# apachepinot/pinot

Measured on NVIDIA B200. Metric: scanned rows/sec for filter+groupby(3 dims,4 aggs) @1/2/4/8 B200; %HBM BW, higher is better.
Workload: dtype f64

## Files before the change

### include/pinot_b200.h

```cpp
#ifndef PINOT_B200_H
#define PINOT_B200_H

#include <stddef.h>
#include <stdint.h>

#ifdef __cplusplus
extern "C" {
#endif

#define PB_OK 0
#define PB_ERR_INVALID (-1)
#define PB_ERR_UNSUPPORTED (-2)
#define PB_ERR_CUDA (-3)
#define PB_ERR_OOM (-4)
#define PB_ERR_STATE (-5)

enum { PB_INT = 0, PB_LONG = 1, PB_FLOAT = 2, PB_DOUBLE = 3, PB_STRING = 4 };

enum { PB_AGG_COUNT = 0, PB_AGG_SUM = 1, PB_AGG_MIN = 2, PB_AGG_MAX = 3, PB_AGG_AVG = 4, PB_AGG_DISTINCTCOUNT = 5 };

enum {
  PB_F_AND = 0, PB_F_OR = 1, PB_F_NOT = 2, PB_F_MATCH_ALL = 3, PB_F_EMPTY = 4,
  PB_F_SCAN_DICT_RANGE = 5,
  PB_F_SCAN_DICT_SET = 6,
// ... 125 lines not shown

int pb_segment_group_remap(pb_segment_group_handle g, const char* column, int32_t segment_index, const int32_t** remap, int32_t* n);

int pb_query_execute(pb_segment_group_handle g, const pb_segment_query* seg_queries, const pb_query_desc* q,
                     pb_result_handle* out);

int32_t pb_result_num_tables(pb_result_handle r);
int64_t pb_result_num_groups(pb_result_handle r, int32_t table);
const int32_t* pb_result_group_dict_ids(pb_result_handle r, int32_t table, int32_t gb);
const void* pb_result_group_key_values(pb_result_handle r, int32_t table, int32_t gb, int32_t* stored_type,
                                       int32_t* entry_bytes);
const double* pb_result_double(pb_result_handle r, int32_t table, int32_t agg);
const int64_t* pb_result_long(pb_result_handle r, int32_t table, int32_t agg);
const int64_t* pb_result_distinct_offsets(pb_result_handle r, int32_t table, int32_t agg);
const int32_t* pb_result_distinct_dict_ids(pb_result_handle r, int32_t table, int32_t agg);
const int64_t* pb_result_distinct_values(pb_result_handle r, int32_t table, int32_t agg);
const pb_exec_stats* pb_result_stats(pb_result_handle r, int32_t table);
double pb_result_device_ms(pb_result_handle r);
double pb_result_scan_kernel_ms(pb_result_handle r);
int pb_result_phase_ms(pb_result_handle r, double* filter_kernel_ms, double* agg_kernel_ms);
int32_t pb_result_kernel_launches(pb_result_handle r);
double pb_result_comm_ms(pb_result_handle r);
int32_t pb_result_in_place_columns(pb_result_handle r);
int pb_result_host_timing(pb_result_handle r, double* out8);
void pb_result_free(pb_result_handle r);

int pb_result_device_buffer(pb_result_handle r, int32_t which, int32_t agg, void** device_ptr, int64_t* num_elements);
int pb_result_merge_gathered(pb_result_handle r, const void* gathered_device_ptr, int32_t n_ranks);
int pb_result_finalize(pb_result_handle r);
void* pb_result_stream(pb_result_handle r);
int pb_result_wait(pb_result_handle r);

int pb_host_register(const void* ptr, size_t bytes);
int pb_host_unregister(const void* ptr);

#ifdef __cplusplus
}
#endif
#endif
```

### pinot_b200/csrc/pb_device.cuh

```cuda
#pragma once
#include <cuda_runtime.h>
#include <stdint.h>

#define PB_NTHREADS 256
#define PB_NWARPS 8
#define PB_CHUNK_DOCS 1024
#define PB_NSTAGE 2
#define PB_MAX_LEAVES 16
#define PB_MAX_NODES 32
#define PB_MAX_GROUP_BY 16
#define PB_MAX_AGGS 16
#define PB_MAX_SCAN_SLOTS 8
#define PB_MAX_AGG_FILTERS 8
#define PB_MAX_AF_LEAVES 16
#define PB_MAX_AF_NODES 48
#define PB_SPARSE_MAX 128
#define PB_OUT_CAP 256
#define PB_CAND_CAP 512
#define PB_SET_SMEM_BYTES 8192

enum { L_TRUE = 0, L_FALSE = 1, L_DICT_RANGE = 2, L_DICT_SET = 3, L_RAW_RANGE_I = 4, L_RAW_RANGE_F = 5,
       L_RAW_SET = 6, L_BITMAP = 7 };
enum { N_LEAF = 0, N_AND = 1, N_OR = 2, N_NOT = 3 };
enum { T_KEYLESS = 0, T_DENSE = 1, T_HASH = 2 };
// ... 105 lines not shown
  unsigned long long* docs_matched;
  uint32_t* first_doc;
  uint32_t num_groups_limit;
  uint32_t limit_active;
};

struct DevQuery {
  int32_t n_segs;
  int32_t n_group_by;
  int32_t n_aggs;
  int32_t table_mode;
  int32_t agg_op[PB_MAX_AGGS];
  int32_t agg_filter_of[PB_MAX_AGGS];
  int32_t n_agg_filters;
  int32_t pad_f;
  int32_t slot_off[PB_MAX_SCAN_SLOTS];
  int32_t stage_bytes;
  int32_t set_cache_bytes;
  int32_t use_tma;
  int32_t generic;
  uint64_t n_units;
  uint64_t n_docs_total;
  int32_t match_all;
  int32_t pad_p;
  int32_t sparse_max;
  int32_t cand_bytes;
  uint64_t unit_lo;
  int32_t phase;
  int32_t st_slots;
  int32_t st_replicas;
  int32_t out_cap, cand_cap;
  uint64_t st_min_docs;
  uint32_t* match_list;
  unsigned long long* match_count;
  const unsigned int* any_limit;
  const DevSegQuery* segs;
  DevTable* tables;
};

__device__ __forceinline__ uint32_t pb_bswap32(uint32_t x) { return __byte_perm(x, 0, 0x0123); }

__device__ __forceinline__ long long pb_enc_f64(double v) {
  long long b = __double_as_longlong(v);
  return b >= 0 ? b : (b ^ 0x7fffffffffffffffLL);
}
__host__ __device__ __forceinline__ double pb_dec_f64(long long e) {
  long long b = e >= 0 ? e : (e ^ 0x7fffffffffffffffLL);
// ... 895 lines not shown
          for (uint32_t b0 = 0; b0 < n_pass; b0 += 32) {
            const uint32_t idx = b0 + (uint32_t)lane;
            bool alive = idx < n_pass;
            const uint32_t off = alive ? (uint32_t)cl[idx] : 0u;
            const uint32_t doc = (uint32_t)unit_doc0 + off;
            for (int i = 0; i < n_cand_leaves; i++) {
              if (alive) alive = pb_leaf_test_doc(sq.leaves[H->flat_leaf[H->n_dense + i]], set_cache, doc);
              if (!__any_sync(0xffffffffu, alive)) break;
            }
            const uint32_t bal = __ballot_sync(0xffffffffu, alive);
            if (bal) {
              const uint32_t n = (uint32_t)__popc(bal);
              if (out_n + n > OUT_CAP) flush_out();
              if (alive) ob[out_n + __popc(bal & lt)] = gunit0 + off;
              out_n += n;
              matched += n;
            }
          }
        }
        __syncwarp();
      }
    }
    flush_out();
    if (lane == 0 && matched) pb_red_add_u64(Q.tables[sq.table].docs_matched, matched);
  }
}

#define PB_AGG_MAX_SEGS_SMEM 1024

template <int MIN_CTAS>
__global__ void __launch_bounds__(PB_NTHREADS, MIN_CTAS) pb_agg_kernel(const __grid_constant__ DevQuery Q) {
  extern __shared__ __align__(128) uint8_t smem_raw[];
  const int tid = threadIdx.x, lane = tid & 31, warp = tid >> 5;
  __shared__ unsigned long long s_doc_base[PB_AGG_MAX_SEGS_SMEM + 1];
  __shared__ unsigned long long s_red_u64[PB_NWARPS];
  __shared__ double s_red_f64[PB_NWARPS];
  __shared__ long long s_red_i64[PB_NWARPS];
  __shared__ int s_table0;
  const int n_segs = Q.n_segs;
  const int n_smem = n_segs < PB_AGG_MAX_SEGS_SMEM ? n_segs : PB_AGG_MAX_SEGS_SMEM;
  for (int i = tid; i < n_smem; i += PB_NTHREADS) s_doc_base[i] = Q.segs[i].doc_base;
  KeylessAcc ka;
  ka.sum = nullptr; ka.mm = nullptr; ka.cnt = nullptr;
  const long long ENC_POS_INF = 0x7ff0000000000000LL;
  const long long ENC_NEG_INF = (long long)0xfff0000000000000ULL ^ 0x7fffffffffffffffLL;
  const bool keyless = Q.table_mode == T_KEYLESS;
  if (keyless) {
// ... 192 lines not shown
    for (int a = 0; a < Q.n_aggs; a++) {
      if (st.fc_of[a] >= 0) {
        unsigned long long fc = 0;
        for (uint32_t r = 0; r < R; r++) { SmemTable z = st; z.base = smem0 + r * (uint32_t)rep_bytes; fc += pb_sh_ld_u32(z.fcnt(st.fc_of[a], i)); }
        if (fc) pb_red_add_u64(&t.fcnt[a][i], fc);
      }
      if (st.acc_of[a] < 0) continue;
      const int op = Q.agg_op[a];
      if (op == 1 || op == 4) {
        double v = 0.0;
        for (uint32_t r = 0; r < R; r++) { SmemTable z = st; z.base = smem0 + r * (uint32_t)rep_bytes; v += __longlong_as_double((long long)pb_sh_ld_u64(z.acc(st.acc_of[a], i))); }
        pb_red_add_f64(&t.sum[a][i], v);
      } else {
        long long m = 0x7fffffffffffffffLL;
        for (uint32_t r = 0; r < R; r++) { SmemTable z = st; z.base = smem0 + r * (uint32_t)rep_bytes; const long long o = (long long)pb_sh_ld_u64(z.acc(st.acc_of[a], i)); m = o < m ? o : m; }
        if (m != 0x7fffffffffffffffLL) pb_red_min_s64(&t.mm[a][i], m);
      }
    }
  }
}

struct DevRowKey { uint32_t off, bits; uint64_t mult; const int32_t* remap; };
struct DevRowAgg { uint32_t off, width, type, exact_int; };
struct DevRowSeg {
  const uint32_t* rows;
  uint64_t doc_base;
  int32_t table, pad;
  DevRowKey keys[PB_MAX_GROUP_BY];
  DevRowAgg aggs[PB_MAX_AGGS];
};
#define PB_ROWS_SMEM_SEGS 16

template <int RW>
__global__ void __launch_bounds__(PB_AGG_SMEM_THREADS, 1) pb_agg_rows_kernel(const __grid_constant__ DevQuery Q, const DevRowSeg* __restrict__ gsegs) {
  extern __shared__ __align__(128) uint8_t smem_raw[];
  __shared__ DevRowSeg s_segs[PB_ROWS_SMEM_SEGS];
  __shared__ unsigned long long s_doc_base[PB_AGG_MAX_SEGS_SMEM + 1];
  const int tid = threadIdx.x, warp = tid >> 5;
  const int n_segs = Q.n_segs, nG = Q.n_group_by, nA = Q.n_aggs;
  const int n_smem = n_segs < PB_AGG_MAX_SEGS_SMEM ? n_segs : PB_AGG_MAX_SEGS_SMEM;
  for (int i = tid; i < n_smem; i += PB_AGG_SMEM_THREADS) s_doc_base[i] = gsegs[i].doc_base;
  const bool segs_in_smem = n_segs <= PB_ROWS_SMEM_SEGS;
  if (segs_in_smem) {
    const uint32_t* src = reinterpret_cast<const uint32_t*>(gsegs);
    uint32_t* dst = reinterpret_cast<uint32_t*>(s_segs);
    for (int i = tid; i < (int)(sizeof(DevRowSeg) / 4) * n_segs; i += PB_AGG_SMEM_THREADS) dst[i] = src[i];
  }
  const DevRowSeg* segs = segs_in_smem ? s_segs : gsegs;
  const unsigned long long n = Q.match_all ? Q.n_docs_total : *Q.match_count;
  const uint32_t S = (uint32_t)Q.st_slots, R = (uint32_t)(Q.st_replicas > 0 ? Q.st_replicas : 1);
  SmemTable st;
  st.S = S;
  int n_acc = 0;
  for (int a = 0; a < PB_MAX_AGGS; a++) {
    const int op = a < nA ? Q.agg_op[a] : 0;
    st.acc_of[a] = (a < nA && op >= 1 && op <= 4) ? (int8_t)n_acc++ : (int8_t)-1;
    st.fc_of[a] = -1;
  }
  st.n_fc = 0;
  const size_t rep_bytes = pb_smem_table_bytes(S, 0, n_acc);
  const uint32_t smem0 = pb_smem_u32(smem_raw);
  st.base = smem0 + ((uint32_t)warp & (R - 1)) * (uint32_t)rep_bytes;
  const bool use_smem = S > 0 && n >= Q.st_min_docs;
  if (use_smem) {
    for (uint32_t r = 0; r < R; r++) {
      SmemTable z = st; z.base = smem0 + r * (uint32_t)rep_bytes;
      for (uint32_t i = tid; i < S; i += PB_AGG_SMEM_THREADS) pb_sh_st_u32(z.cnt(i), 0u);
      for (int a = 0; a < nA; a++) {
        if (st.acc_of[a] < 0) continue;
        const unsigned long long init = (Q.agg_op[a] == 1 || Q.agg_op[a] == 4) ? 0ull : 0x7fffffffffffffffull;
        for (uint32_t i = tid; i < S; i += PB_AGG_SMEM_THREADS) pb_sh_st_u64(z.acc(st.acc_of[a], i), init);
      }
    }
  }
  __syncthreads();

  auto process = [&](unsigned long long gdoc, const uint32_t (&w)[RW], const DevRowSeg& sg) {
    auto field = [&](uint32_t off, uint32_t bits) -> uint32_t {
      const uint32_t wi = off >> 5, sh = off & 31u;
      uint32_t hi = w[0], lo = RW > 1 ? w[1 % RW] : 0u;
#pragma unroll
      for (int k = 1; k < RW; k++) if (wi == (uint32_t)k) { hi = w[k]; lo = k + 1 < RW ? w[(k + 1) % RW] : 0u; }
      return __funnelshift_l(lo, hi, sh) >> (32u - bits);
    };
    uint64_t slot = 0;
    for (int j = 0; j < nG; j++) {
      const DevRowKey& k = sg.keys[j];
      uint32_t id = field(k.off, k.bits);
      if (k.remap) id = (uint32_t)__ldg(k.remap + id);
      slot += (uint64_t)id * k.mult;
    }
    auto value_of = [&](int a) -> double {
      const DevRowAgg& g = sg.aggs[a];
      const uint32_t w0 = field(g.off, 32u);
      if (g.width == 4) return g.type == 2 ? (double)__uint_as_float(w0) : (double)(int32_t)w0;
      const unsigned long long u = ((unsigned long long)w0 << 32) | field(g.off + 32u, 32u);
      return g.type == 3 ? __longlong_as_double((long long)u) : (double)(long long)u;
    };
    auto ivalue_of = [&](int a) -> long long {
      const DevRowAgg& g = sg.aggs[a];
      const uint32_t w0 = field(g.off, 32u);
      if (g.width == 4) return (long long)(int32_t)w0;
      return (long long)(((unsigned long long)w0 << 32) | field(g.off + 32u, 32u));
    };
    if (use_smem) {
      const uint32_t sl = (uint32_t)slot;
      pb_sh_add_u32(st.cnt(sl), 1u);
// ... 39 lines not shown
  };
  auto seg_of = [&](unsigned long long gdoc) -> int {
    int lo = 0, hi = n_segs - 1;
    while (lo < hi) {
      const int mid = (lo + hi + 1) >> 1;
      const unsigned long long b = mid < PB_AGG_MAX_SEGS_SMEM ? s_doc_base[mid] : gsegs[mid].doc_base;
      if (b <= gdoc) lo = mid; else hi = mid - 1;
    }
    return lo;
  };
  auto load_row = [&](const DevRowSeg& sg, unsigned long long gdoc, uint32_t (&w)[RW]) {
    const uint32_t* __restrict__ row = sg.rows + (gdoc - sg.doc_base) * (unsigned long long)RW;
    if (RW == 2) { const uint2 v = __ldg(reinterpret_cast<const uint2*>(row)); w[0] = v.x; w[1 % RW] = v.y; }
    else {
#pragma unroll
      for (int q4 = 0; q4 < RW / 4; q4++) {
        const uint4 v = __ldg(reinterpret_cast<const uint4*>(row) + q4);
        w[(4 * q4) % RW] = v.x; w[(4 * q4 + 1) % RW] = v.y; w[(4 * q4 + 2) % RW] = v.z; w[(4 * q4 + 3) % RW] = v.w;
      }
    }
#pragma unroll
    for (int k = 0; k < RW; k++) w[k] = pb_bswap32(w[k]);
  };
  const unsigned long long stride = (unsigned long long)gridDim.x * PB_AGG_SMEM_THREADS;
  for (unsigned long long i = (unsigned long long)blockIdx.x * PB_AGG_SMEM_THREADS + tid; i < n; i += 2 * stride) {
    const bool two = i + stride < n;
    const unsigned long long gdoc0 = Q.match_all ? i : (unsigned long long)__ldg(Q.match_list + i);
    const unsigned long long gdoc1 = !two ? gdoc0 : (Q.match_all ? i + stride : (unsigned long long)__ldg(Q.match_list + i + stride));
    const DevRowSeg& sg0 = segs[seg_of(gdoc0)];
    const DevRowSeg& sg1 = segs[seg_of(gdoc1)];
    uint32_t w0[RW], w1[RW];
    load_row(sg0, gdoc0, w0);
    load_row(sg1, gdoc1, w1);
    process(gdoc0, w0, sg0);
    if (two) process(gdoc1, w1, sg1);
  }
  if (!use_smem) return;
  __syncthreads();
  const DevTable& t = Q.tables[0];
  for (uint32_t i = tid; i < S; i += PB_AGG_SMEM_THREADS) {
    unsigned long long c = 0;
    for (uint32_t r = 0; r < R; r++) { SmemTable z = st; z.base = smem0 + r * (uint32_t)rep_bytes; c += pb_sh_ld_u32(z.cnt(i)); }
    if (c == 0) continue;
    pb_red_add_u64(&t.rowcnt[i], c);
    for (int a = 0; a < nA; a++) {
      if (st.acc_of[a] < 0) continue;
      const int op = Q.agg_op[a];
      if ((op == 1 || op == 4) && segs[0].aggs[a].exact_int) {
        long long v = 0;
        for (uint32_t r = 0; r < R; r++) { SmemTable z = st; z.base = smem0 + r * (uint32_t)rep_bytes; v += (long long)pb_sh_ld_u64(z.acc(st.acc_of[a], i)); }
        pb_red_add_f64(&t.sum[a][i], (double)v);
      } else if (op == 1 || op == 4) {
        double v = 0.0;
        for (uint32_t r = 0; r < R; r++) { SmemTable z = st; z.base = smem0 + r * (uint32_t)rep_bytes; v += __longlong_as_double((long long)pb_sh_ld_u64(z.acc(st.acc_of[a], i))); }
        pb_red_add_f64(&t.sum[a][i], v);
      } else {
        long long m = 0x7fffffffffffffffLL;
        for (uint32_t r = 0; r < R; r++) { SmemTable z = st; z.base = smem0 + r * (uint32_t)rep_bytes; const long long o = (long long)pb_sh_ld_u64(z.acc(st.acc_of[a], i)); m = o < m ? o : m; }
// ... 654 lines not shown
```

### pinot_b200/csrc/pb_engine.cu

```cuda
#include "../../include/pinot_b200.h"
#include "pb_device.cuh"
#include "pb_filter_spec.h"

#include <dlfcn.h>
#include <nccl.h>

#include <algorithm>
#include <chrono>
#include <cmath>
#include <cstdarg>
#include <cstdio>
#include <cstring>
#include <map>
#include <memory>
#include <mutex>
#include <string>
#include <unordered_set>
#include <vector>

static thread_local char g_err[1024];
static int fail(int code, const char* fmt, ...) {
  va_list ap;
  va_start(ap, fmt);
  vsnprintf(g_err, sizeof g_err, fmt, ap);
// ... 886 lines not shown
  DevTable dev;
  int64_t num_groups = 0;
  HostArr slots, rows;
  std::vector<HostArr> dbl, lng, key_ids, key_vals, dc_off, dc_ids;
  std::vector<int> key_type, key_eb;
  std::vector<uint64_t> dset_cap;
  std::vector<HostArr> dc_vals;
  pb_exec_stats stats{};
  uint64_t out_cap = 0;
};

struct pb_result_s {
  pb_group_s* group = nullptr;
  cudaStream_t stream = nullptr;
  int n_gb = 0, n_aggs = 0;
  int table_mode = 0;
  bool combine = false, finalized = false;
  unsigned long long* d_seg_stats = nullptr;
  int n_agg_filters = 0;
  bool count_all = false;
  std::vector<int> agg_filter_of;
  int waves = 1;
  int in_place_columns = 0;
  std::vector<int> agg_op;
  std::vector<std::string> gb_names, agg_cols;
  std::vector<TableMeta> tables;
  std::vector<void*> dev_allocs;
  void* scratch = nullptr; size_t scratch_cap = 0;
  unsigned long long* d_counters = nullptr;
  HostArr h_counters;
  int n_distinct_cols = 0;
  int n_scan_leaves_total = 0;
  std::vector<int64_t> seg_scan_leaves;
  double device_ms = 0, scan_ms = 0;
  double host_us[8] = {0};
  int launches = 0;
  cudaEvent_t ev0 = nullptr, ev1 = nullptr, evm = nullptr, ev2 = nullptr, ev3 = nullptr;
  StreamSet sset;
  bool match_all = false;
  double filter_ms = 0, agg_ms = 0;
  unsigned long long* span_i64 = nullptr; int64_t span_i64_n = 0;
  double* span_f64 = nullptr; int64_t span_f64_n = 0;
  long long* span_mm = nullptr; int64_t span_mm_n = 0;
  uint8_t* block = nullptr; int64_t block_bytes = 0, block_sum_off = 0, block_dc_off = 0, block_mm_off = 0;
  unsigned long long fingerprint = 0;
  int merged_ranks = 1;
// ... 940 lines not shown
  uint32_t* d_bitmaps = nullptr;
  if (bitmap_words_total) {
    CU(cudaMallocAsync((void**)&d_bitmaps, 4 * bitmap_words_total, st)); r->dev_allocs.push_back(d_bitmaps);
    CU(cudaMemsetAsync(d_bitmaps, 0, 4 * bitmap_words_total, st));
  }

  DevQuery* hq = nullptr;
  DevQuery* dq = ar.put<DevQuery>(nullptr, 1, &hq);
  DevSegQuery* hsegs = nullptr;
  DevSegQuery* dsegs = ar.put<DevSegQuery>(nullptr, (size_t)n_segs, &hsegs);
  DevTable* htabs = nullptr;
  DevTable* dtabs = ar.put<DevTable>(nullptr, (size_t)n_tables, &htabs);
  for (int t = 0; t < n_tables; t++) htabs[t] = r->tables[t].dev;

  struct PendingExpand { int kind; const uint8_t* inv; int card; const int32_t* ids; int n_ids; uint32_t* out; uint32_t num_docs; std::vector<int32_t> host_ids; };
  std::vector<PendingExpand> expands;
  int slot_bits_max[PB_MAX_SCAN_SLOTS] = {0};
  int set_cache_max = 0;
  int n_slots_max = 0;
  bool any_cand_leaf = false;
  size_t bm_off = 0;
  r->seg_scan_leaves.assign(n_segs, 0);

  for (int si = 0; si < n_segs; si++) {
    pb_segment_s* s = g->segs[si];
    const pb_segment_query& sq = sqs[si];
    DevSegQuery& ds = hsegs[si];
    ds.num_docs = s->num_docs;
    ds.table = combine ? 0 : si;
    int n_scan = 0, set_smem_used = 0;
    int slot_of_col[PB_MAX_SCAN_SLOTS];
    auto build_program = [&](const pb_filter_node* nodes, int n_nodes, int8_t* node_kind, int8_t* node_arg, DevLeaf* leaves, int max_leaves,
                             int& n_leaves, bool force_gather) -> int {
    for (int n = 0; n < n_nodes; n++) {
      const pb_filter_node& fn = nodes[n];
      if (fn.kind == PB_F_AND || fn.kind == PB_F_OR) {
        if (fn.num_children < 1 || fn.num_children > PB_MAX_LEAVES) return fail(PB_ERR_UNSUPPORTED, "AND/OR with %d children", fn.num_children);
        node_kind[n] = fn.kind == PB_F_AND ? N_AND : N_OR; node_arg[n] = (int8_t)fn.num_children; continue;
      }
      if (fn.kind == PB_F_NOT) { node_kind[n] = N_NOT; node_arg[n] = 1; continue; }
      if (n_leaves >= max_leaves) return fail(PB_ERR_UNSUPPORTED, "more than %d filter leaves", max_leaves);
      DevLeaf& lf = leaves[n_leaves];
      memset(&lf, 0, sizeof lf);
      lf.set_smem_off = -1;
      lf.est_permille = 500;
      node_kind[n] = N_LEAF; node_arg[n] = (int8_t)n_leaves; n_leaves++;
      auto scan_slot = [&](const Column& c) -> int {
        if (force_gather || cand_leaf[si][n]) {
          lf.gather = 1;
          lf.gfwd = c.fwd_staged ? c.d_fwd : c.d_fwd_host;
          lf.g_full_words = c.fwd_staged ? 0xFFFFFFFFu : c.host_full_words;
          lf.g_tail_word = c.fwd_staged ? 0u : c.host_tail_word;
          lf.g_stride_bits = c.bits; lf.g_bit_off = 0;
          if (!c.has_dict) lf.g_stride_bits = 8 * c.raw_width;
          if (c.has_dict && seg_rg[si] && seg_rg[si]->find(fn.column, 0) >= 0) {
            const RowGroup* rg = seg_rg[si];
            lf.gfwd = rg->d_rows; lf.g_full_words = 0xFFFFFFFFu; lf.g_tail_word = 0u;
            lf.g_stride_bits = rg->stride_bits; lf.g_bit_off = rg->bit_off[(size_t)rg->find(fn.column, 0)];
          }
          if (!c.fwd_staged) r->in_place_columns++;
          any_cand_leaf = true;
          return PB_MAX_SCAN_SLOTS;
        }
        for (int k = 0; k < n_scan; k++) if (slot_of_col[k] == fn.column) return k;
        if (n_scan >= PB_MAX_SCAN_SLOTS) return -1;
        slot_of_col[n_scan] = fn.column;
        DevScanCol& sc = ds.scan[n_scan];
        sc.base = c.d_fwd; sc.bits_per_doc = c.has_dict ? c.bits : 8 * c.raw_width; sc.bytes_total = c.d_fwd_bytes;
        slot_bits_max[n_scan] = std::max(slot_bits_max[n_scan], sc.bits_per_doc);
        return n_scan++;
      };
      switch (fn.kind) {
        case PB_F_MATCH_ALL: lf.kind = L_TRUE; break;
        case PB_F_EMPTY: lf.kind = L_FALSE; break;
        case PB_F_SCAN_DICT_RANGE: {
          const Column& c = s->cols[fn.column];
          int64_t lo = std::max<int64_t>(fn.lo, 0), hi = std::min<int64_t>(fn.hi, c.card);
          if (hi <= lo) { lf.kind = L_FALSE; break; }
          if (lo == 0 && hi >= c.card) { lf.kind = L_TRUE; break; }
          lf.kind = L_DICT_RANGE; lf.bits = c.bits; lf.lo = (uint32_t)lo; lf.span = (uint32_t)(hi - lo);
          lf.est_permille = (int32_t)(1000.0 * (double)(hi - lo) / (double)c.card);
          if ((lf.slot = scan_slot(c)) < 0) return fail(PB_ERR_UNSUPPORTED, "more than %d scanned columns", PB_MAX_SCAN_SLOTS);
          r->seg_scan_leaves[si]++;
          break;
        }
        case PB_F_SCAN_DICT_SET: {
          const Column& c = s->cols[fn.column];
          if (fn.num_ids <= 0) { lf.kind = fn.exclusive ? L_TRUE : L_FALSE; break; }
          size_t words = ((size_t)c.card + 31) / 32;
          uint32_t* hbits = nullptr;
          const uint32_t* dbits = ar.put<uint32_t>(nullptr, words, &hbits);
          if (!dbits) return fail(PB_ERR_STATE, "query arena overflow");
          for (int k = 0; k < fn.num_ids; k++) {
            int32_t id = fn.ids[k];
            if (id < 0 || id >= c.card) return fail(PB_ERR_INVALID, "filter node %d: dictId %d out of range", n, id);
            hbits[id >> 5] |= 1u << (id & 31);
          }
          lf.kind = L_DICT_SET; lf.bits = c.bits; lf.exclusive = fn.exclusive ? 1 : 0;
          lf.set_bits = dbits; lf.set_card = c.card;
          { double f = (double)fn.num_ids / (double)c.card; lf.est_permille = (int32_t)(1000.0 * (fn.exclusive ? 1.0 - f : f)); }
          if (!force_gather && set_smem_used + c.card <= PB_SET_SMEM_BYTES) { lf.set_smem_off = set_smem_used; set_smem_used += (c.card + 15) & ~15; }
          if ((lf.slot = scan_slot(c)) < 0) return fail(PB_ERR_UNSUPPORTED, "more than %d scanned columns", PB_MAX_SCAN_SLOTS);
          r->seg_scan_leaves[si]++;
          break;
        }
        case PB_F_SCAN_RAW_RANGE: {
          const Column& c = s->cols[fn.column];
          lf.raw_width = c.raw_width; lf.data_type = c.type;
          if (c.type == PB_INT || c.type == PB_LONG) { lf.kind = L_RAW_RANGE_I; lf.ilo = fn.lo; lf.ihi = fn.hi; }
          else { lf.kind = L_RAW_RANGE_F; lf.dlo = fn.dlo; lf.dhi = fn.dhi; lf.dlo_incl = fn.dlo_inclusive; lf.dhi_incl = fn.dhi_inclusive; }
          if ((lf.slot = scan_slot(c)) < 0) return fail(PB_ERR_UNSUPPORTED, "more than %d scanned columns", PB_MAX_SCAN_SLOTS);
          r->seg_scan_leaves[si]++;
          break;
        }
        case PB_F_SCAN_RAW_SET: {
          const Column& c = s->cols[fn.column];
          if (fn.num_raw_values <= 0) { lf.kind = fn.exclusive ? L_TRUE : L_FALSE; break; }
          lf.kind = L_RAW_SET; lf.raw_width = c.raw_width; lf.data_type = c.type; lf.exclusive = fn.exclusive ? 1 : 0;
          lf.raw_set = ar.put<int64_t>(fn.raw_values, (size_t)fn.num_raw_values);
          lf.n_raw_set = fn.num_raw_values;
          if (!lf.raw_set) return fail(PB_ERR_STATE, "query arena overflow");
          if ((lf.slot = scan_slot(c)) < 0) return fail(PB_ERR_UNSUPPORTED, "more than %d scanned columns", PB_MAX_SCAN_SLOTS);
          r->seg_scan_leaves[si]++;
          break;
        }
// ... 25 lines not shown
            std::vector<uint8_t> tmp(8 + blob_len);
            uint32_t o0 = 8, o1 = (uint32_t)(8 + blob_len);
            tmp[0] = o0 >> 24; tmp[1] = o0 >> 16; tmp[2] = o0 >> 8; tmp[3] = (uint8_t)o0;
            tmp[4] = o1 >> 24; tmp[5] = o1 >> 16; tmp[6] = o1 >> 8; tmp[7] = (uint8_t)o1;
            memcpy(tmp.data() + 8, blob, blob_len);
            const uint8_t* dblob = ar.put<uint8_t>(tmp.data(), tmp.size());
            static const int32_t zero_id = 0;
            const int32_t* dids = ar.put<int32_t>(&zero_id, 1);
            if (!dblob || !dids) return fail(PB_ERR_STATE, "query arena overflow");
            expands.push_back({0, dblob, 1, dids, 1, bm, (uint32_t)s->num_docs, std::vector<int32_t>(1, 0)});
          }
          break;
        }
        default: return fail(PB_ERR_INVALID, "filter node %d: unknown kind %d", n, fn.kind);
      }
      if (lf.gather) lf.slot = -1;
    }
    return PB_OK;
    };
    ds.n_nodes = sq.num_filter_nodes;
    {
      int nl = 0;
      if ((rc = build_program(sq.filter, sq.num_filter_nodes, ds.node_kind, ds.node_arg, ds.leaves, PB_MAX_LEAVES, nl, false))) return rc;
    }
    ds.n_agg_filters = nF;
    {
      int nl = 0, nn = 0;
      for (int f = 0; f < nF; f++) {
        ds.af_begin[f] = nn;
        if (nn + sq.agg_filter_nodes[f] > PB_MAX_AF_NODES) return fail(PB_ERR_UNSUPPORTED, "FILTER clauses have more than %d nodes", PB_MAX_AF_NODES);
        if ((rc = build_program(sq.agg_filters[f], sq.agg_filter_nodes[f], ds.af_node_kind + nn, ds.af_node_arg + nn, ds.af_leaves, PB_MAX_AF_LEAVES, nl, true))) return rc;
        nn += sq.agg_filter_nodes[f];
      }
      for (int f = nF; f <= PB_MAX_AGG_FILTERS; f++) ds.af_begin[f] = nn;
      ds.af_docs = d_seg_stats ? d_seg_stats + (size_t)si * (1 + PB_MAX_AGG_FILTERS) : nullptr;
    }
    ds.n_scan = n_scan;
    set_cache_max = std::max(set_cache_max, set_smem_used);
    n_slots_max = std::max(n_slots_max, n_scan);
    r->n_scan_leaves_total += (int)r->seg_scan_leaves[si];

    const TableMeta& tm = r->tables[ds.table];
    uint64_t mult = 1;
    for (int j = 0; j < nG; j++) {
      const Column& c = s->cols[gcol[si][j]];
      DevKeyCol& kc = ds.keys[j];
// ... 16 lines not shown
      if (acol[si][a] < 0) continue;
      const Column& c = s->cols[acol[si][a]];
      DevAggCol& ac = ds.aggs[a];
      ac.fwd = c.fwd_staged ? c.d_fwd : c.d_fwd_host; ac.n_full_words = c.fwd_staged ? 0xFFFFFFFFu : c.host_full_words;
      ac.tail_word = c.fwd_staged ? 0u : c.host_tail_word; if (!c.fwd_staged) r->in_place_columns++;
      ac.dict_f64 = c.d_dict_f64; ac.bits = c.bits; ac.raw_width = c.has_dict ? 0 : c.raw_width; ac.data_type = c.type;
      ac.stride_bits = c.has_dict ? c.bits : 8 * c.raw_width; ac.bit_off = 0;
      if (c.has_dict && seg_rg[si]) {
        const RowGroup* rg = seg_rg[si];
        const int fv = q->aggregations[a].op != PB_AGG_DISTINCTCOUNT ? rg->find(acol[si][a], 1) : -1, fi = rg->find(acol[si][a], 0);
        if (fv >= 0) {
          ac.fwd = rg->d_rows; ac.n_full_words = 0xFFFFFFFFu; ac.tail_word = 0u;
          ac.raw_width = c.entry_bytes; ac.stride_bits = rg->stride_bits; ac.bit_off = rg->bit_off[(size_t)fv];
        } else if (fi >= 0) {
          ac.fwd = rg->d_rows; ac.n_full_words = 0xFFFFFFFFu; ac.tail_word = 0u;
          ac.stride_bits = rg->stride_bits; ac.bit_off = rg->bit_off[(size_t)fi];
        }
      }
      ac.remap = (combine && adict[a]) ? adict[a]->d_remap[si] : nullptr;
    }
  }

  const DevRowSeg* d_row_segs = nullptr;
  int rows_rw = 0;
  {
    static const bool rows_on = []() { const char* e = getenv("PB_AGG_ROWS"); return !e || atoi(e) != 0; }();
    bool ok = rows_on && table_mode == T_DENSE && nF == 0 && nG > 0 && n_segs > 0;
    for (int si = 0; si < n_segs && ok; si++) {
      const RowGroup* rg = seg_rg[si];
      if (!rg || (rows_rw && rows_rw != rg->stride_bits / 32)) { ok = false; break; }
      rows_rw = rg->stride_bits / 32;
      for (int j = 0; j < nG && ok; j++) if (rg->find(gcol[si][j], 0) < 0) ok = false;
      for (int a = 0; a < nA && ok; a++) {
        const int op = q->aggregations[a].op;
        if (op == PB_AGG_COUNT) continue;
        if (op == PB_AGG_DISTINCTCOUNT || rg->find(acol[si][a], 1) < 0) ok = false;
      }
    }
    if (ok) {
      DevRowSeg* h_rs = nullptr;
      d_row_segs = ar.put<DevRowSeg>(nullptr, (size_t)n_segs, &h_rs);
      if (!d_row_segs) return fail(PB_ERR_STATE, "query arena overflow");
      for (int si = 0; si < n_segs; si++) {
        const RowGroup* rg = seg_rg[si];
        const pb_segment_s* sg = g->segs[si];
        DevRowSeg& rs = h_rs[si];
        rs.rows = reinterpret_cast<const uint32_t*>(rg->d_rows);
        rs.table = hsegs[si].table;
        for (int j = 0; j < nG; j++) {
          const DevKeyCol& kc = hsegs[si].keys[j];
          rs.keys[j].off = (uint32_t)rg->bit_off[(size_t)rg->find(gcol[si][j], 0)];
          rs.keys[j].bits = (uint32_t)sg->cols[gcol[si][j]].bits;
          rs.keys[j].mult = kc.mult; rs.keys[j].remap = kc.remap;
        }
        for (int a = 0; a < nA; a++) {
          if (q->aggregations[a].op == PB_AGG_COUNT) continue;
          const Column& c = sg->cols[acol[si][a]];
          rs.aggs[a].off = (uint32_t)rg->bit_off[(size_t)rg->find(acol[si][a], 1)];
          rs.aggs[a].width = (uint32_t)c.entry_bytes; rs.aggs[a].type = (uint32_t)c.type; rs.aggs[a].exact_int = 0;
        }
      }
      static const bool exact_on = []() { const char* e = getenv("PB_AGG_EXACT_INT"); return !e || atoi(e) != 0; }();
      uint64_t docs_all = 0;
      for (int si = 0; si < n_segs; si++) docs_all += (uint64_t)g->segs[si]->num_docs;
      for (int a = 0; a < nA && exact_on; a++) {
        const int op = q->aggregations[a].op;
        if (op != PB_AGG_SUM && op != PB_AGG_AVG) continue;
        bool exact = true;
        for (int si = 0; si < n_segs && exact; si++) {
          const Column& c = g->segs[si]->cols[acol[si][a]];
          if (!c.has_dict || c.card <= 0 || (c.type != PB_INT && c.type != PB_LONG) || c.h_dict.size() < (size_t)c.card * (size_t)c.entry_bytes) { exact = false; break; }
          const uint8_t* lo = c.h_dict.data(); const uint8_t* hi = c.h_dict.data() + (size_t)(c.card - 1) * (size_t)c.entry_bytes;
          const int64_t vlo = c.type == PB_INT ? (int64_t)(int32_t)be32(lo) : (int64_t)be64(lo);
          const int64_t vhi = c.type == PB_INT ? (int64_t)(int32_t)be32(hi) : (int64_t)be64(hi);
          const uint64_t alo = vlo < 0 ? (uint64_t)0 - (uint64_t)vlo : (uint64_t)vlo, ahi = vhi < 0 ? (uint64_t)0 - (uint64_t)vhi : (uint64_t)vhi;
          const uint64_t bound = std::max<uint64_t>(std::max(alo, ahi), 1);
          if (bound >= (1ull << 53) || docs_all >= (1ull << 53) / bound) exact = false;
        }
        if (exact) for (int si = 0; si < n_segs; si++) h_rs[si].aggs[a].exact_int = 1;
      }
    } else rows_rw = 0;
  }

  int sum_bits = 0;
  for (int k = 0; k < n_slots_max; k++) sum_bits += slot_bits_max[k];
  static const int unit_env = []() { const char* e = getenv("PB_UNIT"); return e ? atoi(e) : 2; }();
  auto stage_bytes_for = [&](int U, int32_t* offs) {
    size_t b = 0;
    for (int k = 0; k < n_slots_max; k++) {
      if (offs) offs[k] = (int32_t)b;
      b += (((size_t)U * PB_CHUNK_DOCS * slot_bits_max[k] / 8 + 16) + 15) & ~(size_t)15;
    }
    return b;
  };
  int U = (unit_env == 1) ? 1 : 2;
  if (U == 2 && stage_bytes_for(2, nullptr) * PB_NSTAGE * PB_NWARPS > 100 * 1024) U = 1;
  int32_t slot_offs[PB_MAX_SCAN_SLOTS] = {0};
  size_t stage_bytes = stage_bytes_for(U, slot_offs);
  if (stage_bytes * PB_NSTAGE * PB_NWARPS > 200 * 1024)
    return fail(PB_ERR_UNSUPPORTED, "scan predicates touch %d bits per row: unit stages do not fit shared memory", sum_bits);
  const uint64_t unit_docs = (uint64_t)U * PB_CHUNK_DOCS;
  uint64_t n_chunks = 0, n_docs_total = 0;
  bool match_all = true;
  for (int si = 0; si < n_segs; si++) {
// ... 80 lines not shown
          for (int a = 0; a < nA; a++) if (in_lane[a]) { in_main[a] = 1; any_main = true; }
          continue;
        }
        lw.docs_w[1 + f] = 1; lw.post_w[1 + f] = lane_cols(in_lane);
      }
      for (int a = 0; a < nA; a++) if (q->agg_filter_of[a] < 0) { in_main[a] = 1; any_main = true; }
      if (any_main || nG > 0) { lw.docs_w[0] = 1; lw.post_w[0] = lane_cols(in_main); }
    }
  }

  hq->n_segs = n_segs; hq->n_group_by = nG; hq->n_aggs = nA; hq->table_mode = table_mode;
  for (int a = 0; a < nA; a++) hq->agg_op[a] = q->aggregations[a].op;
  for (int a = 0; a < PB_MAX_AGGS; a++) hq->agg_filter_of[a] = (nF > 0 && a < nA) ? q->agg_filter_of[a] : -1;
  hq->n_agg_filters = nF;
  for (int k = 0; k < n_slots_max; k++) hq->slot_off[k] = slot_offs[k];
  hq->stage_bytes = (int32_t)stage_bytes;
  hq->set_cache_bytes = set_cache_max;
  hq->out_cap = PB_OUT_CAP; hq->cand_cap = PB_CAND_CAP;
  hq->cand_bytes = any_cand_leaf ? (int32_t)(2 * PB_CAND_CAP * PB_NWARPS) : 0;
  hq->use_tma = (q->flags & PB_Q_NO_TMA) ? 0 : 1;
  hq->generic = (q->flags & PB_Q_GENERIC_KERNEL) ? 1 : 0;
  hq->n_units = n_chunks; hq->segs = dsegs; hq->tables = dtabs;
  hq->n_docs_total = n_docs_total; hq->match_all = match_all ? 1 : 0;
  { static const int sm = []() { const char* e = getenv("PB_SPARSE_MAX"); return e ? atoi(e) : PB_SPARSE_MAX; }(); hq->sparse_max = sm; }
  hq->match_list = d_match_list;
  if (use_smem_table) {
    hq->st_slots = (int32_t)r->tables[0].capacity; hq->st_replicas = st_replicas;
    static const long long min_env = []() { const char* e = getenv("PB_AGG_SMEM_MIN"); return e ? atoll(e) : -1ll; }();
    hq->st_min_docs = min_env >= 0 ? (uint64_t)min_env : 4ull * (uint64_t)ctx->num_sms * r->tables[0].capacity;
  }
  r->fused = fuse; r->smem_table = use_smem_table;
  hq->match_count = reinterpret_cast<unsigned long long*>(d_aux);
  hq->any_limit = reinterpret_cast<const unsigned int*>(d_aux + any_limit_off);
  r->repair_pass = false;
  if (table_mode == T_HASH) for (auto& tm : r->tables) if (tm.dev.limit_active) r->repair_pass = true;

  int n_expand_items = 0;
  for (auto& e : expands) n_expand_items += e.kind == 0 ? e.n_ids : 1;
  const DevExpandItem* d_expand_items = nullptr;
  if (n_expand_items > 0) {
    std::vector<DevExpandItem> items;
    items.reserve((size_t)n_expand_items);
    for (auto& e : expands) {
      if (e.kind == 0) {
        for (int k = 0; k < e.n_ids; k++) {
          DevExpandItem it; memset(&it, 0, sizeof it);
// ... 680 lines not shown
  if (!r) return fail(PB_ERR_INVALID, "null result");
  if (!r->finalized) {
    float ms = 0;
    cudaEventSynchronize(r->ev2);
    cudaEventElapsedTime(&ms, r->ev1, r->evm); r->filter_ms = ms;
    cudaEventElapsedTime(&ms, r->evm, r->ev2); r->agg_ms = ms;
  }
  if (filter_ms) *filter_ms = r->filter_ms;
  if (agg_ms) *agg_ms = r->agg_ms;
  return PB_OK;
}
extern "C" int pb_result_host_timing(pb_result_handle r, double* out8) {
  if (!r || !out8) return fail(PB_ERR_INVALID, "null argument");
  for (int i = 0; i < 8; i++) out8[i] = r->host_us[i];
  return PB_OK;
}
extern "C" int pb_result_wait(pb_result_handle r) {
  if (!r) return fail(PB_ERR_INVALID, "null result");
  for (auto* p : r->parts) if (p->stream) { DeviceGuard dgp(p->ctx); CU(cudaStreamSynchronize(p->stream)); }
  if (r->stream) { DeviceGuard dg(r->ctx); CU(cudaStreamSynchronize(r->stream)); }
  return PB_OK;
}
extern "C" int32_t pb_result_in_place_columns(pb_result_handle r) { return r ? r->in_place_columns : 0; }
extern "C" double pb_result_comm_ms(pb_result_handle r) {
  if (!r || !r->comm_timed) return 0;
  if (r->comm_ms == 0) { float ms = 0; cudaEventSynchronize(r->sset.ev[6]); if (cudaEventElapsedTime(&ms, r->sset.ev[5], r->sset.ev[6]) == cudaSuccess) r->comm_ms = ms; }
  return r->comm_ms;
}

extern "C" int pb_host_register(const void* ptr, size_t bytes) {
  int rc = ensure_init();
  if (rc) return rc;
  DeviceGuard dg(g_all.ctxs[0].get());
  CU(cudaHostRegister(const_cast<void*>(ptr), bytes, cudaHostRegisterPortable | cudaHostRegisterMapped));
  return PB_OK;
}
extern "C" int pb_host_unregister(const void* ptr) {
  CU(cudaHostUnregister(const_cast<void*>(ptr)));
  return PB_OK;
}

extern "C" int pb_result_device_buffer(pb_result_handle r, int32_t which, int32_t agg, void** device_ptr, int64_t* num_elements) {
  if (!r || !device_ptr || !num_elements) return fail(PB_ERR_INVALID, "null argument");
  if (!r->combine || r->tables.size() != 1) return fail(PB_ERR_STATE, "device buffers are exposed for PB_Q_COMBINE results only");
  if (r->table_mode == T_HASH) return fail(PB_ERR_UNSUPPORTED, "hash tables cannot be all-reduced in place");
  TableMeta& tm = r->tables[0];
// ... 61 lines not shown
```

### pinot_b200/native.py

```python
from __future__ import annotations

import ctypes as C
import os
from typing import Dict, List, Optional, Sequence

import numpy as np

from .query import AggOp, QueryContext
from .segment_writer import DataType, Segment

_HERE = os.path.dirname(os.path.abspath(__file__))
LIB_PATH = os.environ.get("PB_LIB_PATH") or os.path.join(_HERE, "libpinot_b200.so")

PB_Q_COMBINE = 1
PB_Q_DEFER_FINALIZE = 2
PB_Q_GENERIC_KERNEL = 4
PB_Q_NO_TMA = 8
PB_Q_GATHER_IN_PLACE = 16
PB_Q_ALL_RANKS = 32
PB_COMM_ID_BYTES = 128


class PbColumnDesc(C.Structure):
    _fields_ = [("name", C.c_char_p), ("stored_type", C.c_int32), ("has_dictionary", C.c_int32),
# ... 99 lines not shown
    l.pb_result_group_dict_ids.restype = C.POINTER(C.c_int32)
    l.pb_result_group_key_values.argtypes = [C.c_void_p, C.c_int32, C.c_int32, C.POINTER(C.c_int32), C.POINTER(C.c_int32)]
    l.pb_result_group_key_values.restype = C.c_void_p
    l.pb_result_double.argtypes = [C.c_void_p, C.c_int32, C.c_int32]
    l.pb_result_double.restype = C.POINTER(C.c_double)
    l.pb_result_long.argtypes = [C.c_void_p, C.c_int32, C.c_int32]
    l.pb_result_long.restype = C.POINTER(C.c_int64)
    l.pb_result_distinct_offsets.argtypes = [C.c_void_p, C.c_int32, C.c_int32]
    l.pb_result_distinct_offsets.restype = C.POINTER(C.c_int64)
    l.pb_result_distinct_dict_ids.argtypes = [C.c_void_p, C.c_int32, C.c_int32]
    l.pb_result_distinct_dict_ids.restype = C.POINTER(C.c_int32)
    l.pb_result_distinct_values.argtypes = [C.c_void_p, C.c_int32, C.c_int32]
    l.pb_result_distinct_values.restype = C.POINTER(C.c_int64)
    l.pb_result_stats.argtypes = [C.c_void_p, C.c_int32]
    l.pb_result_stats.restype = C.POINTER(PbExecStats)
    l.pb_result_device_ms.argtypes = [C.c_void_p]
    l.pb_result_device_ms.restype = C.c_double
    l.pb_result_scan_kernel_ms.argtypes = [C.c_void_p]
    l.pb_result_scan_kernel_ms.restype = C.c_double
    l.pb_result_kernel_launches.argtypes = [C.c_void_p]
    l.pb_result_kernel_launches.restype = C.c_int32
    l.pb_result_in_place_columns.argtypes = [C.c_void_p]
    l.pb_result_in_place_columns.restype = C.c_int32
    l.pb_result_stream.argtypes = [C.c_void_p]
    l.pb_result_stream.restype = C.c_void_p
    l.pb_result_wait.argtypes = [C.c_void_p]
    l.pb_result_merge_gathered.argtypes = [C.c_void_p, C.c_void_p, C.c_int32]
    l.pb_result_phase_ms.argtypes = [C.c_void_p, C.POINTER(C.c_double), C.POINTER(C.c_double)]
    l.pb_result_host_timing.argtypes = [C.c_void_p, C.POINTER(C.c_double)]
    l.pb_host_register.argtypes = [C.c_void_p, C.c_size_t]
    l.pb_host_unregister.argtypes = [C.c_void_p]
    l.pb_result_device_buffer.argtypes = [C.c_void_p, C.c_int32, C.c_int32, C.POINTER(C.c_void_p), C.POINTER(C.c_int64)]
    _lib = l
    return l


class PinotB200Error(RuntimeError):
    def __init__(self, code: int, msg: str):
        super().__init__(f"pinot_b200 error {code}: {msg}")
        self.code = code


def _check(rc: int):
    if rc != 0:
        raise PinotB200Error(rc, lib().pb_last_error().decode("utf-8", "replace"))

# ... 202 lines not shown
        out = {}
        nh = getattr(self.query, "null_handling", False)
        for g, k in enumerate(ks):
            row = []
            for a, agg in enumerate(self.query.aggregations):
                if agg.op in (AggOp.COUNT, AggOp.DISTINCTCOUNT):
                    row.append(int(lng[a][g]))
                elif nh and int(lng[a][g]) == 0:
                    row.append(None)
                elif agg.op == AggOp.AVG:
                    row.append((float(dbl[a][g]), int(lng[a][g])))
                else:
                    row.append(float(dbl[a][g]))
            out[k] = row
        return out


class Result:
    def __init__(self, rh, q: QueryContext, deferred: bool = False):
        self._rh = rh
        self.query = q
        self._finalized = not deferred
        self.in_place_columns = lib().pb_result_in_place_columns(rh)
        if not deferred:
            self._load()

    @property
    def tables(self) -> List[ResultTable]:
        if not self._finalized:
            return []
        return [ResultTable(self._rh, t, self.query, self) for t in range(lib().pb_result_num_tables(self._rh))]

    def _load(self):
        l = lib()
        self._finalized = True
        self.device_ms = l.pb_result_device_ms(self._rh)
        self.scan_kernel_ms = l.pb_result_scan_kernel_ms(self._rh)
        self.kernel_launches = l.pb_result_kernel_launches(self._rh)
        self.in_place_columns = l.pb_result_in_place_columns(self._rh)

    def device_buffer(self, which: int, agg: int = 0):
        p, n = C.c_void_p(), C.c_int64()
        _check(lib().pb_result_device_buffer(self._rh, which, agg, C.byref(p), C.byref(n)))
        return p.value, n.value

    def merge_gathered(self, gathered_ptr: int, n_ranks: int):
# ... 160 lines not shown
```

Baseline: 537.5 billion.

## Push dictionary filter leaves into row-layout aggregation kernel as residual predicates

Candidate dictionary range/set filter leaves are evaluated inside the row-group aggregation kernel, reading the packed row words it already loads, instead of being gathered in the filter kernel. The filter program is rebuilt as an AND over the remaining leaves, and the docs-matched count moves to the agg kernel through a warp-reduced counter. This aims to cut a separate column gather in the filter stage, at the cost of extra per-row predicate work and a rewrite of the filter tree that assumes a flat AND structure.

```diff
diff --git a/include/pinot_b200.h b/include/pinot_b200.h
--- a/include/pinot_b200.h
+++ b/include/pinot_b200.h
@@ -171,6 +171,7 @@
 int32_t pb_result_kernel_launches(pb_result_handle r);
 double pb_result_comm_ms(pb_result_handle r);
 int32_t pb_result_in_place_columns(pb_result_handle r);
+int32_t pb_result_residual_leaves(pb_result_handle r);
 int pb_result_host_timing(pb_result_handle r, double* out8);
 void pb_result_free(pb_result_handle r);
 
diff --git a/pinot_b200/csrc/pb_device.cuh b/pinot_b200/csrc/pb_device.cuh
--- a/pinot_b200/csrc/pb_device.cuh
+++ b/pinot_b200/csrc/pb_device.cuh
@@ -151,7 +151,7 @@
   uint64_t n_units;
   uint64_t n_docs_total;
   int32_t match_all;
-  int32_t pad_p;
+  int32_t agg_counts_docs;
   int32_t sparse_max;
   int32_t cand_bytes;
   uint64_t unit_lo;
@@ -1093,7 +1093,7 @@
       }
     }
     flush_out();
-    if (lane == 0 && matched) pb_red_add_u64(Q.tables[sq.table].docs_matched, matched);
+    if (lane == 0 && matched && !Q.agg_counts_docs) pb_red_add_u64(Q.tables[sq.table].docs_matched, matched);
   }
 }
 
@@ -1332,14 +1332,31 @@
 
 struct DevRowKey { uint32_t off, bits; uint64_t mult; const int32_t* remap; };
 struct DevRowAgg { uint32_t off, width, type, exact_int; };
+struct DevRowLeaf {
+  uint32_t off, bits;
+  uint32_t lo, span;
+  const uint32_t* set;
+  uint32_t excl, pad;
+};
+#define PB_ROWS_MAX_LEAVES 4
 struct DevRowSeg {
   const uint32_t* rows;
   uint64_t doc_base;
-  int32_t table, pad;
+  int32_t table, n_leaves;
   DevRowKey keys[PB_MAX_GROUP_BY];
   DevRowAgg aggs[PB_MAX_AGGS];
+  DevRowLeaf leaves[PB_ROWS_MAX_LEAVES];
 };
 #define PB_ROWS_SMEM_SEGS 16
+
+template <int RW>
+__device__ __forceinline__ uint32_t pb_row_field(const uint32_t (&w)[RW], uint32_t off, uint32_t bits) {
+  const uint32_t wi = off >> 5, sh = off & 31u;
+  uint32_t hi = w[0], lo = RW > 1 ? w[1 % RW] : 0u;
+#pragma unroll
+  for (int k = 1; k < RW; k++) if (wi == (uint32_t)k) { hi = w[k]; lo = k + 1 < RW ? w[(k + 1) % RW] : 0u; }
+  return __funnelshift_l(lo, hi, sh) >> (32u - bits);
+}
 
 template <int RW>
 __global__ void __launch_bounds__(PB_AGG_SMEM_THREADS, 1) pb_agg_rows_kernel(const __grid_constant__ DevQuery Q, const DevRowSeg* __restrict__ gsegs) {
@@ -1386,13 +1403,7 @@
   __syncthreads();
 
   auto process = [&](unsigned long long gdoc, const uint32_t (&w)[RW], const DevRowSeg& sg) {
-    auto field = [&](uint32_t off, uint32_t bits) -> uint32_t {
-      const uint32_t wi = off >> 5, sh = off & 31u;
-      uint32_t hi = w[0], lo = RW > 1 ? w[1 % RW] : 0u;
-#pragma unroll
-      for (int k = 1; k < RW; k++) if (wi == (uint32_t)k) { hi = w[k]; lo = k + 1 < RW ? w[(k + 1) % RW] : 0u; }
-      return __funnelshift_l(lo, hi, sh) >> (32u - bits);
-    };
+    auto field = [&](uint32_t off, uint32_t bits) -> uint32_t { return pb_row_field<RW>(w, off, bits); };
     uint64_t slot = 0;
     for (int j = 0; j < nG; j++) {
       const DevRowKey& k = sg.keys[j];
@@ -1478,6 +1489,21 @@
 #pragma unroll
     for (int k = 0; k < RW; k++) w[k] = pb_bswap32(w[k]);
   };
+  auto passes = [&](const uint32_t (&w)[RW], const DevRowSeg& sg) -> bool {
+    for (int k = 0; k < sg.n_leaves; k++) {
+      const DevRowLeaf& l = sg.leaves[k];
+      const uint32_t id = pb_row_field<RW>(w, l.off, l.bits);
+      const bool ok = l.set ? (((__ldg(l.set + (id >> 5)) >> (id & 31)) & 1u) ^ l.excl) != 0u : (id - l.lo) < l.span;
+      if (!ok) return false;
+    }
+    return true;
+  };
+  int cnt_table = 0;
+  uint32_t cnt = 0;
+  auto count = [&](int table) {
+    if (table != cnt_table && cnt) { pb_red_add_u64(Q.tables[cnt_table].docs_matched, cnt); cnt = 0; }
+    cnt_table = table; cnt++;
+  };
   const unsigned long long stride = (unsigned long long)gridDim.x * PB_AGG_SMEM_THREADS;
   for (unsigned long long i = (unsigned long long)blockIdx.x * PB_AGG_SMEM_THREADS + tid; i < n; i += 2 * stride) {
     const bool two = i + stride < n;
@@ -1488,8 +1514,21 @@
     uint32_t w0[RW], w1[RW];
     load_row(sg0, gdoc0, w0);
     load_row(sg1, gdoc1, w1);
-    process(gdoc0, w0, sg0);
-    if (two) process(gdoc1, w1, sg1);
+    const bool ok0 = passes(w0, sg0), ok1 = two && passes(w1, sg1);
+    if (ok0) process(gdoc0, w0, sg0);
+    if (ok1) process(gdoc1, w1, sg1);
+    if (Q.agg_counts_docs) { if (ok0) count(sg0.table); if (ok1) count(sg1.table); }
+  }
+  if (Q.agg_counts_docs) {
+    const unsigned has = __ballot_sync(0xffffffffu, cnt != 0);
+    if (has) {
+      const int leader = __ffs(has) - 1;
+      const int t0 = __shfl_sync(0xffffffffu, cnt_table, leader);
+      if (__all_sync(0xffffffffu, cnt == 0 || cnt_table == t0)) {
+        const uint32_t sum = __reduce_add_sync(0xffffffffu, cnt);
+        if ((tid & 31) == leader) pb_red_add_u64(Q.tables[t0].docs_matched, sum);
+      } else if (cnt) pb_red_add_u64(Q.tables[cnt_table].docs_matched, cnt);
+    }
   }
   if (!use_smem) return;
   __syncthreads();
diff --git a/pinot_b200/csrc/pb_engine.cu b/pinot_b200/csrc/pb_engine.cu
--- a/pinot_b200/csrc/pb_engine.cu
+++ b/pinot_b200/csrc/pb_engine.cu
@@ -932,6 +932,7 @@
   std::vector<int> agg_filter_of;
   int waves = 1;
   int in_place_columns = 0;
+  int residual_leaves = 0;
   std::vector<int> agg_op;
   std::vector<std::string> gb_names, agg_cols;
   std::vector<TableMeta> tables;
@@ -1918,6 +1919,28 @@
   size_t bm_off = 0;
   r->seg_scan_leaves.assign(n_segs, 0);
 
+  int rows_rw = 0;
+  bool rows_ok = false;
+  {
+    static const bool rows_on = []() { const char* e = getenv("PB_AGG_ROWS"); return !e || atoi(e) != 0; }();
+    rows_ok = rows_on && table_mode == T_DENSE && nF == 0 && nG > 0 && n_segs > 0;
+    for (int si = 0; si < n_segs && rows_ok; si++) {
+      const RowGroup* rg = seg_rg[si];
+      if (!rg || (rows_rw && rows_rw != rg->stride_bits / 32)) { rows_ok = false; break; }
+      rows_rw = rg->stride_bits / 32;
+      for (int j = 0; j < nG && rows_ok; j++) if (rg->find(gcol[si][j], 0) < 0) rows_ok = false;
+      for (int a = 0; a < nA && rows_ok; a++) {
+        const int op = q->aggregations[a].op;
+        if (op == PB_AGG_COUNT) continue;
+        if (op == PB_AGG_DISTINCTCOUNT || rg->find(acol[si][a], 1) < 0) rows_ok = false;
+      }
+    }
+    if (!rows_ok) rows_rw = 0;
+  }
+  static const bool residual_on = []() { const char* e = getenv("PB_AGG_RESIDUAL"); return !e || atoi(e) != 0; }();
+  std::vector<std::vector<DevRowLeaf>> residual(n_segs);
+  r->residual_leaves = 0;
+
   for (int si = 0; si < n_segs; si++) {
     pb_segment_s* s = g->segs[si];
     const pb_segment_query& sq = sqs[si];
@@ -1926,6 +1949,7 @@
     ds.table = combine ? 0 : si;
     int n_scan = 0, set_smem_used = 0;
     int slot_of_col[PB_MAX_SCAN_SLOTS];
+    std::vector<char> residual_node((size_t)std::max(sq.num_filter_nodes, 0), 0);
     auto build_program = [&](const pb_filter_node* nodes, int n_nodes, int8_t* node_kind, int8_t* node_arg, DevLeaf* leaves, int max_leaves,
                              int& n_leaves, bool force_gather) -> int {
     for (int n = 0; n < n_nodes; n++) {
@@ -1941,6 +1965,15 @@
       lf.set_smem_off = -1;
       lf.est_permille = 500;
       node_kind[n] = N_LEAF; node_arg[n] = (int8_t)n_leaves; n_leaves++;
+      const int residual_field = (!force_gather && rows_ok && residual_on && cand_leaf[si][n] && residual[si].size() < PB_ROWS_MAX_LEAVES &&
+                                  (fn.kind == PB_F_SCAN_DICT_RANGE || fn.kind == PB_F_SCAN_DICT_SET)) ? seg_rg[si]->find(fn.column, 0) : -1;
+      auto make_residual = [&](const Column& c, const uint32_t* set) {
+        DevRowLeaf rl; memset(&rl, 0, sizeof rl);
+        rl.off = (uint32_t)seg_rg[si]->bit_off[(size_t)residual_field]; rl.bits = (uint32_t)c.bits;
+        rl.lo = lf.lo; rl.span = lf.span; rl.set = set; rl.excl = (uint32_t)lf.exclusive;
+        residual[si].push_back(rl);
+        residual_node[n] = 1;
+      };
       auto scan_slot = [&](const Column& c) -> int {
         if (force_gather || cand_leaf[si][n]) {
           lf.gather = 1;
@@ -1976,7 +2009,8 @@
           if (lo == 0 && hi >= c.card) { lf.kind = L_TRUE; break; }
           lf.kind = L_DICT_RANGE; lf.bits = c.bits; lf.lo = (uint32_t)lo; lf.span = (uint32_t)(hi - lo);
           lf.est_permille = (int32_t)(1000.0 * (double)(hi - lo) / (double)c.card);
-          if ((lf.slot = scan_slot(c)) < 0) return fail(PB_ERR_UNSUPPORTED, "more than %d scanned columns", PB_MAX_SCAN_SLOTS);
+          if (residual_field >= 0) make_residual(c, nullptr);
+          else if ((lf.slot = scan_slot(c)) < 0) return fail(PB_ERR_UNSUPPORTED, "more than %d scanned columns", PB_MAX_SCAN_SLOTS);
           r->seg_scan_leaves[si]++;
           break;
         }
@@ -1995,8 +2029,11 @@
           lf.kind = L_DICT_SET; lf.bits = c.bits; lf.exclusive = fn.exclusive ? 1 : 0;
           lf.set_bits = dbits; lf.set_card = c.card;
           { double f = (double)fn.num_ids / (double)c.card; lf.est_permille = (int32_t)(1000.0 * (fn.exclusive ? 1.0 - f : f)); }
-          if (!force_gather && set_smem_used + c.card <= PB_SET_SMEM_BYTES) { lf.set_smem_off = set_smem_used; set_smem_used += (c.card + 15) & ~15; }
-          if ((lf.slot = scan_slot(c)) < 0) return fail(PB_ERR_UNSUPPORTED, "more than %d scanned columns", PB_MAX_SCAN_SLOTS);
+          if (residual_field >= 0) make_residual(c, dbits);
+          else {
+            if (!force_gather && set_smem_used + c.card <= PB_SET_SMEM_BYTES) { lf.set_smem_off = set_smem_used; set_smem_used += (c.card + 15) & ~15; }
+            if ((lf.slot = scan_slot(c)) < 0) return fail(PB_ERR_UNSUPPORTED, "more than %d scanned columns", PB_MAX_SCAN_SLOTS);
+          }
           r->seg_scan_leaves[si]++;
           break;
         }
@@ -2068,6 +2105,19 @@
     {
       int nl = 0;
       if ((rc = build_program(sq.filter, sq.num_filter_nodes, ds.node_kind, ds.node_arg, ds.leaves, PB_MAX_LEAVES, nl, false))) return rc;
+      if (!residual[si].empty()) {
+        int kept = 0;
+        for (int n = 0; n + 1 < sq.num_filter_nodes; n++) {
+          if (residual_node[n]) continue;
+          ds.leaves[kept] = ds.leaves[ds.node_arg[n]];
+          ds.node_kind[kept] = N_LEAF; ds.node_arg[kept] = (int8_t)kept;
+          kept++;
+        }
+        ds.node_kind[kept] = N_AND; ds.node_arg[kept] = (int8_t)kept;
+        ds.n_nodes = kept + 1;
+        for (int l = kept; l < nl; l++) memset(&ds.leaves[l], 0, sizeof(DevLeaf));
+        r->residual_leaves += (int)residual[si].size();
+      }
     }
     ds.n_agg_filters = nF;
     {
@@ -2130,22 +2180,8 @@
   }
 
   const DevRowSeg* d_row_segs = nullptr;
-  int rows_rw = 0;
-  {
-    static const bool rows_on = []() { const char* e = getenv("PB_AGG_ROWS"); return !e || atoi(e) != 0; }();
-    bool ok = rows_on && table_mode == T_DENSE && nF == 0 && nG > 0 && n_segs > 0;
-    for (int si = 0; si < n_segs && ok; si++) {
-      const RowGroup* rg = seg_rg[si];
-      if (!rg || (rows_rw && rows_rw != rg->stride_bits / 32)) { ok = false; break; }
-      rows_rw = rg->stride_bits / 32;
-      for (int j = 0; j < nG && ok; j++) if (rg->find(gcol[si][j], 0) < 0) ok = false;
-      for (int a = 0; a < nA && ok; a++) {
-        const int op = q->aggregations[a].op;
-        if (op == PB_AGG_COUNT) continue;
-        if (op == PB_AGG_DISTINCTCOUNT || rg->find(acol[si][a], 1) < 0) ok = false;
-      }
-    }
-    if (ok) {
+  if (rows_ok) {
+    {
       DevRowSeg* h_rs = nullptr;
       d_row_segs = ar.put<DevRowSeg>(nullptr, (size_t)n_segs, &h_rs);
       if (!d_row_segs) return fail(PB_ERR_STATE, "query arena overflow");
@@ -2167,6 +2203,8 @@
           rs.aggs[a].off = (uint32_t)rg->bit_off[(size_t)rg->find(acol[si][a], 1)];
           rs.aggs[a].width = (uint32_t)c.entry_bytes; rs.aggs[a].type = (uint32_t)c.type; rs.aggs[a].exact_int = 0;
         }
+        rs.n_leaves = (int32_t)residual[si].size();
+        for (int k = 0; k < rs.n_leaves; k++) rs.leaves[k] = residual[si][(size_t)k];
       }
       static const bool exact_on = []() { const char* e = getenv("PB_AGG_EXACT_INT"); return !e || atoi(e) != 0; }();
       uint64_t docs_all = 0;
@@ -2187,7 +2225,7 @@
         }
         if (exact) for (int si = 0; si < n_segs; si++) h_rs[si].aggs[a].exact_int = 1;
       }
-    } else rows_rw = 0;
+    }
   }
 
   int sum_bits = 0;
@@ -2314,6 +2352,7 @@
   hq->generic = (q->flags & PB_Q_GENERIC_KERNEL) ? 1 : 0;
   hq->n_units = n_chunks; hq->segs = dsegs; hq->tables = dtabs;
   hq->n_docs_total = n_docs_total; hq->match_all = match_all ? 1 : 0;
+  hq->agg_counts_docs = r->residual_leaves > 0 ? 1 : 0;
   { static const int sm = []() { const char* e = getenv("PB_SPARSE_MAX"); return e ? atoi(e) : PB_SPARSE_MAX; }(); hq->sparse_max = sm; }
   hq->match_list = d_match_list;
   if (use_smem_table) {
@@ -3040,6 +3079,7 @@
   return PB_OK;
 }
 extern "C" int32_t pb_result_in_place_columns(pb_result_handle r) { return r ? r->in_place_columns : 0; }
+extern "C" int32_t pb_result_residual_leaves(pb_result_handle r) { return r ? r->residual_leaves : 0; }
 extern "C" double pb_result_comm_ms(pb_result_handle r) {
   if (!r || !r->comm_timed) return 0;
   if (r->comm_ms == 0) { float ms = 0; cudaEventSynchronize(r->sset.ev[6]); if (cudaEventElapsedTime(&ms, r->sset.ev[5], r->sset.ev[6]) == cudaSuccess) r->comm_ms = ms; }
diff --git a/pinot_b200/native.py b/pinot_b200/native.py
--- a/pinot_b200/native.py
+++ b/pinot_b200/native.py
@@ -145,6 +145,8 @@
     l.pb_result_kernel_launches.restype = C.c_int32
     l.pb_result_in_place_columns.argtypes = [C.c_void_p]
     l.pb_result_in_place_columns.restype = C.c_int32
+    l.pb_result_residual_leaves.argtypes = [C.c_void_p]
+    l.pb_result_residual_leaves.restype = C.c_int32
     l.pb_result_stream.argtypes = [C.c_void_p]
     l.pb_result_stream.restype = C.c_void_p
     l.pb_result_wait.argtypes = [C.c_void_p]
@@ -393,6 +395,7 @@
         self.query = q
         self._finalized = not deferred
         self.in_place_columns = lib().pb_result_in_place_columns(rh)
+        self.residual_leaves = lib().pb_result_residual_leaves(rh)
         if not deferred:
             self._load()
 
```

After: 579.1 billion (median of 6 runs). +7.7%, better.
